# tuna2134/sbv2-api

Measured on NVIDIA B200. Metric: audio-sec/sec, higher is better.
Workload: dtype f16 operands / f32 accumulate on tcgen05 (decoder, flow; text encoder with two-term fp16 splits); f32 elsewhere

## Files before the change

### sbv2-api_b200/csrc/flow_attention_tc.cu

```cuda
#include <cuda_fp16.h>
#include <math_constants.h>

#include "kernels.h"

namespace sbv2 {
namespace {

constexpr int QT = 128, KT = 128, D = 96, DP = D / 8, RP = 16;
constexpr uint32_t TILE_BYTES = DP * KT * 16;
constexpr uint32_t P_BYTES = (KT / 8) * QT * 16;
constexpr uint32_t PREL_BYTES = (RP / 8) * QT * 16;
constexpr uint32_t REL_BYTES = DP * RP * 16;
constexpr int TM_O = 0, TM_SREL = 96, TM_S = 128 , TM_COLS = 512;
constexpr int NKV = 3;
constexpr int NSM_WARPS = 8;

__device__ __forceinline__ uint32_t smem_u32(const void* p) { return (uint32_t)__cvta_generic_to_shared(p); }
__device__ __forceinline__ void mbar_init(uint32_t bar, uint32_t count) {
  asm volatile("mbarrier.init.shared::cta.b64 [%0], %1;" ::"r"(bar), "r"(count));
}
__device__ __forceinline__ void mbar_expect_tx(uint32_t bar, uint32_t bytes) {
  asm volatile("mbarrier.arrive.expect_tx.shared::cta.b64 _, [%0], %1;" ::"r"(bar), "r"(bytes) : "memory");
}
__device__ __forceinline__ void mbar_arrive(uint32_t bar) {
  asm volatile("mbarrier.arrive.shared::cta.b64 _, [%0];" ::"r"(bar) : "memory");
}
__device__ __forceinline__ void mbar_wait(uint32_t bar, uint32_t parity) {
  asm volatile(
      "{\n"
      ".reg .pred P1;\n"
      "LAB_WAIT:\n"
      "mbarrier.try_wait.parity.shared::cta.b64 P1, [%0], %1, %2;\n"
      "@P1 bra DONE;\n"
      "bra LAB_WAIT;\n"
      "DONE:\n"
      "}\n" ::"r"(bar),
      "r"(parity), "r"(0x989680u)
      : "memory");
}
__device__ __forceinline__ void bulk_g2s(uint32_t dst, const void* src, uint32_t bytes, uint32_t bar) {
  asm volatile("cp.async.bulk.shared::cluster.global.mbarrier::complete_tx::bytes [%0], [%1], %2, [%3];" ::"r"(dst), "l"(src),
               "r"(bytes), "r"(bar)
               : "memory");
}
__device__ __forceinline__ void tc_fence_before() { asm volatile("tcgen05.fence::before_thread_sync;" ::: "memory"); }
__device__ __forceinline__ void tc_fence_after() { asm volatile("tcgen05.fence::after_thread_sync;" ::: "memory"); }
__device__ __forceinline__ void tc_commit(uint32_t bar) {
  asm volatile("tcgen05.commit.cta_group::1.mbarrier::arrive::one.shared::cluster.b64 [%0];" ::"r"(bar) : "memory");
}
__device__ __forceinline__ void tc_mma_f16(uint32_t tmem_d, uint64_t adesc, uint64_t bdesc, uint32_t idesc, uint32_t accumulate) {
  asm volatile(
      "{\n"
      ".reg .pred p;\n"
      "setp.ne.b32 p, %4, 0;\n"
      "tcgen05.mma.cta_group::1.kind::f16 [%0], %1, %2, %3, p;\n"
      "}\n" ::"r"(tmem_d),
      "l"(adesc), "l"(bdesc), "r"(idesc), "r"(accumulate)
      : "memory");
}
__device__ __forceinline__ void tc_ld32(uint32_t taddr, uint32_t* v) {
  asm volatile(
      "tcgen05.ld.sync.aligned.32x32b.x32.b32 "
      "{%0,%1,%2,%3,%4,%5,%6,%7,%8,%9,%10,%11,%12,%13,%14,%15,%16,%17,%18,%19,%20,%21,%22,%23,%24,%25,%26,%27,%28,%29,%30,%31}, [%32];"
      : "=r"(v[0]), "=r"(v[1]), "=r"(v[2]), "=r"(v[3]), "=r"(v[4]), "=r"(v[5]), "=r"(v[6]), "=r"(v[7]), "=r"(v[8]), "=r"(v[9]),
        "=r"(v[10]), "=r"(v[11]), "=r"(v[12]), "=r"(v[13]), "=r"(v[14]), "=r"(v[15]), "=r"(v[16]), "=r"(v[17]), "=r"(v[18]),
        "=r"(v[19]), "=r"(v[20]), "=r"(v[21]), "=r"(v[22]), "=r"(v[23]), "=r"(v[24]), "=r"(v[25]), "=r"(v[26]), "=r"(v[27]),
        "=r"(v[28]), "=r"(v[29]), "=r"(v[30]), "=r"(v[31])
      : "r"(taddr)
      : "memory");
}
__device__ __forceinline__ void tc_ld16(uint32_t taddr, uint32_t* v) {
  asm volatile(
      "tcgen05.ld.sync.aligned.32x32b.x16.b32 {%0,%1,%2,%3,%4,%5,%6,%7,%8,%9,%10,%11,%12,%13,%14,%15}, [%16];"
      : "=r"(v[0]), "=r"(v[1]), "=r"(v[2]), "=r"(v[3]), "=r"(v[4]), "=r"(v[5]), "=r"(v[6]), "=r"(v[7]), "=r"(v[8]), "=r"(v[9]),
        "=r"(v[10]), "=r"(v[11]), "=r"(v[12]), "=r"(v[13]), "=r"(v[14]), "=r"(v[15])
      : "r"(taddr)
      : "memory");
}
__device__ __forceinline__ void tc_wait_ld() { asm volatile("tcgen05.wait::ld.sync.aligned;" ::: "memory"); }
__device__ __forceinline__ uint32_t elect_one_sync() {
  uint32_t pred = 0;
  asm volatile(
      "{\n"
      ".reg .b32 %%rx;\n"
      ".reg .pred %%px;\n"
      "elect.sync %%rx|%%px, %1;\n"
      "@%%px mov.s32 %0, 1;\n"
      "}\n"
      : "+r"(pred)
      : "r"(0xffffffffu));
  return pred;
}
__device__ __forceinline__ float ex2_approx(float x) {
  float y;
  asm("ex2.approx.ftz.f32 %0, %1;" : "=f"(y) : "f"(x));
  return y;
}
__device__ __forceinline__ uint64_t make_desc(uint32_t saddr, uint32_t lbo_bytes, uint32_t sbo_bytes) {
  return (uint64_t)((saddr >> 4) & 0x3FFF) | ((uint64_t)((lbo_bytes >> 4) & 0x3FFF) << 16) | ((uint64_t)((sbo_bytes >> 4) & 0x3FFF) << 32) |
         ((uint64_t)1 << 46);
}
constexpr uint32_t idesc_f16(int n, int b_mn_major) {
  return (1u << 4) | ((uint32_t)b_mn_major << 16) | ((uint32_t)(n >> 3) << 17) | ((uint32_t)(128 >> 4) << 24);
}

#define ATRACE(ev, i)                                                                                   \
  do {                                                                                                   \
    if (trace != nullptr && blockIdx.x == 0 && blockIdx.y == 0 && blockIdx.z == 0 && (i) < 64) trace[(i) * 8 + (ev)] = clock64(); \
  } while (0)

__global__ void __launch_bounds__(288, 1) flow_attention_tc_kernel(__half* out, const __half* qkv, const __half* rel_k_p,
                                                                    const __half* rel_v_p, int heads, int window, PlanarSegs s,
                                                                    long long* trace) {
  extern __shared__ __align__(128) uint8_t smem[];
  const int warp = __shfl_sync(0xffffffffu, (int)(threadIdx.x >> 5), 0), lane = threadIdx.x & 31;
  const int b = s.order ? s.order[blockIdx.z] : (int)blockIdx.z, h = blockIdx.y;
  const int len = s.len[b];
  const int q0 = blockIdx.x * QT;
  if (q0 >= len) return;
  const long long pbase = s.pstart[b];
  const int n_kt = (len + KT - 1) / KT;

  const uint32_t sQ = smem_u32(smem);
  const uint32_t sK0 = sQ + TILE_BYTES;
  const uint32_t sV0 = sK0 + NKV * TILE_BYTES;
  const uint32_t sP = sV0 + NKV * TILE_BYTES;
  const uint32_t sPrel = sP + P_BYTES;
  const uint32_t sEk = sPrel + PREL_BYTES;
  const uint32_t sEv = sEk + REL_BYTES;
  const uint32_t sBar = sEv + REL_BYTES;
  const uint32_t bar_q = sBar, bar_kv = sBar + 8 , bar_kvfree = sBar + 40 , bar_s = sBar + 72 ,
                 bar_sfree = sBar + 88 , bar_p = sBar + 104, bar_pfree = sBar + 112, bar_done = sBar + 120;
  const uint32_t tmem_slot = sBar + 128;
  float* ml_x = reinterpret_cast<float*>(smem + (sBar - sQ) + 256);
  volatile uint32_t* tmem_slot_ptr = reinterpret_cast<volatile uint32_t*>(smem + (tmem_slot - sQ));

  if (threadIdx.x == 0) {
    mbar_init(bar_q, 1);
    for (int i = 0; i < NKV; ++i) {
      mbar_init(bar_kv + 8 * i, 1);
      mbar_init(bar_kvfree + 8 * i, 1);
    }
    mbar_init(bar_s, 1);
    mbar_init(bar_s + 8, 1);
    mbar_init(bar_sfree, 32 * NSM_WARPS);
    mbar_init(bar_sfree + 8, 32 * NSM_WARPS);
    mbar_init(bar_p, 32 * NSM_WARPS);
    mbar_init(bar_pfree, 1);
    mbar_init(bar_done, 1);
    asm volatile("fence.mbarrier_init.release.cluster;" ::: "memory");
  }
  if (warp == NSM_WARPS) {
    asm volatile("tcgen05.alloc.cta_group::1.sync.aligned.shared::cta.b32 [%0], %1;" ::"r"(tmem_slot), "r"((uint32_t)TM_COLS) : "memory");
    asm volatile("tcgen05.relinquish_alloc_permit.cta_group::1.sync.aligned;" ::: "memory");
  }
  if (threadIdx.x < 128) {
    const uint4 z = make_uint4(0, 0, 0, 0);
    *reinterpret_cast<uint4*>(smem + (sPrel - sQ) + threadIdx.x * 16) = z;
    *reinterpret_cast<uint4*>(smem + (sPrel - sQ) + QT * 16 + threadIdx.x * 16) = z;
  }
  asm volatile("fence.proxy.async.shared::cta;" ::: "memory");
  tc_fence_before();
  __syncthreads();
  tc_fence_after();
  const uint32_t tmem = *tmem_slot_ptr;
  pdl_launch_dependents();
  pdl_wait();

  const int q_plane0 = h * DP, k_plane0 = heads * DP + h * DP, v_plane0 = 2 * heads * DP + h * DP;
  const int n_tiles_total = 2 * n_kt;

  if (warp == NSM_WARPS) {
    auto load_tile = [&](int i) {
      const int buf = i % NKV;
      const uint32_t par = ((i / NKV) & 1) ^ 1;
      const int kt = i < n_kt ? i : i - n_kt;
      const bool with_v = i >= n_kt;
      const long long row0 = pbase + (long long)kt * KT;
      mbar_wait(bar_kvfree + 8 * buf, par);
      if (lane == 0) mbar_expect_tx(bar_kv + 8 * buf, with_v ? 2 * TILE_BYTES : TILE_BYTES);
      __syncwarp();
      if (lane < DP) {
        bulk_g2s(sK0 + buf * TILE_BYTES + lane * KT * 16, qkv + (size_t)(k_plane0 + lane) * s.plane_stride + row0 * 8, KT * 16,
                 bar_kv + 8 * buf);
      } else if (lane < 2 * DP && with_v) {
        const int pl = lane - DP;
        bulk_g2s(sV0 + buf * TILE_BYTES + pl * KT * 16, qkv + (size_t)(v_plane0 + pl) * s.plane_stride + row0 * 8, KT * 16,
                 bar_kv + 8 * buf);
      }
      __syncwarp();
    };
    if (elect_one_sync()) {
      mbar_expect_tx(bar_q, TILE_BYTES + 2 * REL_BYTES);
      for (int pl = 0; pl < DP; ++pl)
        bulk_g2s(sQ + pl * QT * 16, qkv + (size_t)(q_plane0 + pl) * s.plane_stride + (pbase + q0) * 8, QT * 16, bar_q);
      bulk_g2s(sEk, rel_k_p, REL_BYTES, bar_q);
      bulk_g2s(sEv, rel_v_p, REL_BYTES, bar_q);
    }
    __syncwarp();
    for (int i = 0; i < NKV && i < n_tiles_total; ++i) load_tile(i);
    mbar_wait(bar_q, 0);
    tc_fence_after();
    const uint64_t dq = make_desc(sQ, QT * 16, 128);
    const uint64_t dek = make_desc(sEk, RP * 16, 128);
    const uint64_t dp = make_desc(sP, QT * 16, 128);
    const uint64_t dprel = make_desc(sPrel, QT * 16, 128);
    const uint64_t dev = make_desc(sEv, 128, RP * 16);
    constexpr uint32_t ID_S = idesc_f16(KT, 0), ID_REL = idesc_f16(RP, 0), ID_O = idesc_f16(D, 1);
    if (elect_one_sync()) {
      for (int k = 0; k < D / 16; ++k)
        tc_mma_f16(tmem + TM_SREL, dq + (uint64_t)(k * 2 * QT), dek + (uint64_t)(k * 2 * RP), ID_REL, k > 0 ? 1u : 0u);
    }
    __syncwarp();
    auto issue_s = [&](int i) {
      const int sb = i & 1, kb = i % NKV;
      mbar_wait(bar_kv + 8 * kb, (i / NKV) & 1);
      if (lane == 0) ATRACE(0, i);
      mbar_wait(bar_sfree + 8 * sb, ((i >> 1) & 1) ^ 1);
      tc_fence_after();
      if (lane == 0) ATRACE(1, i);
      const uint64_t dk = make_desc(sK0 + kb * TILE_BYTES, KT * 16, 128);
      if (elect_one_sync()) {
        for (int k = 0; k < D / 16; ++k)
          tc_mma_f16(tmem + TM_S + sb * KT, dq + (uint64_t)(k * 2 * QT), dk + (uint64_t)(k * 2 * KT), ID_S, k > 0 ? 1u : 0u);
        tc_commit(bar_s + 8 * sb);
        if (i < n_kt) tc_commit(bar_kvfree + 8 * kb);
      }
      __syncwarp();
    };
    issue_s(0);
    for (int i = 0; i < n_tiles_total; ++i) {
      const int kb = i % NKV;
      if (i + 1 < n_tiles_total) issue_s(i + 1);
      if (i >= n_kt) {
        const int j = i - n_kt;
        mbar_wait(bar_p, j & 1);
        tc_fence_after();
        if (lane == 0) ATRACE(2, i);
        const uint64_t dv = make_desc(sV0 + kb * TILE_BYTES, 128, KT * 16);
        if (elect_one_sync()) {
          for (int k = 0; k < KT / 16; ++k)
            tc_mma_f16(tmem + TM_O, dp + (uint64_t)(k * 2 * QT), dv + (uint64_t)(k * 16), ID_O, (j > 0 || k > 0) ? 1u : 0u);
          tc_commit(bar_pfree);
          tc_commit(bar_kvfree + 8 * kb);
        }
        __syncwarp();
      }
      if (i + NKV < n_tiles_total) load_tile(i + NKV);
      if (lane == 0) ATRACE(3, i);
    }
    if (elect_one_sync()) {
      tc_mma_f16(tmem + TM_O, dprel, dev, ID_O, 1u);
      tc_commit(bar_done);
    }
    __syncwarp();
  } else {
    const int quarter = warp & 3, half = warp >> 2;
    const int row = quarter * 32 + lane;
    const int qi = q0 + row;
    const uint32_t lane_addr = tmem + ((uint32_t)(quarter * 32) << 16);
    const float c_scale = 1.4426950408889634f / sqrtf((float)D);
    float srel[9];
    {
      mbar_wait(bar_s, 0);
      tc_fence_after();
      uint32_t v[16];
      tc_ld16(lane_addr + TM_SREL, v);
      tc_wait_ld();
#pragma unroll
      for (int r = 0; r < 9; ++r) srel[r] = __uint_as_float(v[r]) * c_scale;
    }
    float m2 = -CUDART_INF_F, l = 0.f, mb = 0.f;
    uint8_t* prow = smem + (sP - sQ) + row * 16;
    uint8_t* prel_row = smem + (sPrel - sQ) + row * 16;
    auto pass_a = [&](const float* x, float c) {
      float mx = x[0];
#pragma unroll
      for (int e = 1; e < 32; ++e) mx = fmaxf(mx, x[e]);
      m2 = fmaxf(m2, mx * c);
    };
    auto pass_b_store = [&](const float* x, float c, int c32, float* pv) {
      float sum = 0.f;
#pragma unroll
      for (int e = 0; e < 32; ++e) {
        pv[e] = ex2_approx(fmaf(x[e], c, -mb));
        sum += pv[e];
      }
      l += sum;
#pragma unroll
      for (int q = 0; q < 4; ++q) {
        uint4 u;
        __half2* uh = reinterpret_cast<__half2*>(&u);
#pragma unroll
        for (int e = 0; e < 4; ++e) uh[e] = __floats2half2_rn(pv[q * 8 + 2 * e], pv[q * 8 + 2 * e + 1]);
        *reinterpret_cast<uint4*>(prow + (size_t)(c32 * 4 + q) * QT * 16) = u;
      }
    };
    for (int i = 0; i < n_tiles_total; ++i) {
      const bool pass_b = i >= n_kt;
      const int kt = pass_b ? i - n_kt : i;
      const int k0 = kt * KT;
      const int buf = i & 1;
      if (i > 0) {
        mbar_wait(bar_s + 8 * buf, (i >> 1) & 1);
        tc_fence_after();
      }
      if (threadIdx.x == 0) ATRACE(4, i);
      if (i == n_kt) {
        ml_x[(half * QT + row) * 2] = m2;
        asm volatile("bar.sync 1, %0;" ::"r"(32 * NSM_WARPS) : "memory");
        mb = fmaxf(m2, ml_x[((half ^ 1) * QT + row) * 2]);
      }
      if (pass_b && kt > 0) mbar_wait(bar_pfree, (kt - 1) & 1);
      if (threadIdx.x == 0) ATRACE(5, i);
#pragma unroll 1
      for (int cc = 0; cc < KT / 64; ++cc) {
        const int c = half * (KT / 64) + cc;
        const int kc0 = k0 + c * 32;
        if (kc0 >= len) {
          if (pass_b) {
            const uint4 z = make_uint4(0, 0, 0, 0);
#pragma unroll
            for (int q = 0; q < 4; ++q) *reinterpret_cast<uint4*>(prow + (size_t)(c * 4 + q) * QT * 16) = z;
          }
          continue;
        }
        uint32_t v[32];
        tc_ld32(lane_addr + TM_S + buf * KT + c * 32, v);
        tc_wait_ld();
        float* x = reinterpret_cast<float*>(v);
        const int j0 = kc0 - qi + 4;
        const bool band = j0 <= 8 && j0 + 31 >= 0;
        const bool tail = kc0 + 32 > len;
        if (!__any_sync(0xffffffffu, band) && !tail) {
          if (!pass_b) {
            pass_a(x, c_scale);
          } else {
            float pv[32];
            pass_b_store(x, c_scale, c, pv);
          }
          continue;
        }
#pragma unroll
        for (int e = 0; e < 32; ++e) {
          const int r = j0 + e;
          float add = 0.f;
#pragma unroll
          for (int rr = 0; rr < 9; ++rr) add = (r == rr) ? srel[rr] : add;
          x[e] = (kc0 + e < len) ? fmaf(x[e], c_scale, add) : -CUDART_INF_F;
        }
        if (!pass_b) {
          pass_a(x, 1.0f);
        } else {
          float pv[32];
          pass_b_store(x, 1.0f, c, pv);
#pragma unroll
          for (int rr = 0; rr < 9; ++rr) {
            const int e = rr - j0;
            float val = 0.f;
#pragma unroll
            for (int ee = 0; ee < 32; ++ee) val = (e == ee) ? pv[ee] : val;
            if (e >= 0 && e < 32) *reinterpret_cast<__half*>(prel_row + (size_t)(rr >> 3) * QT * 16 + (rr & 7) * 2) = __float2half_rn(val);
          }
        }
      }
      if (threadIdx.x == 0) ATRACE(6, i);
      tc_fence_before();
      mbar_arrive(bar_sfree + 8 * buf);
      if (pass_b) {
        asm volatile("fence.proxy.async.shared::cta;" ::: "memory");
        mbar_arrive(bar_p);
      }
    }
    ml_x[(half * QT + row) * 2 + 1] = l;
    asm volatile("bar.sync 1, %0;" ::"r"(32 * NSM_WARPS) : "memory");
    const float inv_l = 1.0f / (l + ml_x[((half ^ 1) * QT + row) * 2 + 1]);
    mbar_wait(bar_done, 0);
    tc_fence_after();
#pragma unroll 1
    for (int c = half * 2; c < (half == 0 ? 2 : D / 32); ++c) {
      uint32_t v[32];
      tc_ld32(lane_addr + TM_O + c * 32, v);
      tc_wait_ld();
      if (qi < len) {
#pragma unroll
        for (int q = 0; q < 4; ++q) {
          uint4 u;
          __half2* uh = reinterpret_cast<__half2*>(&u);
#pragma unroll
          for (int e = 0; e < 4; ++e)
            uh[e] = __floats2half2_rn(__uint_as_float(v[q * 8 + 2 * e]) * inv_l, __uint_as_float(v[q * 8 + 2 * e + 1]) * inv_l);
          *reinterpret_cast<uint4*>(out + (size_t)(h * DP + c * 4 + q) * s.plane_stride + (pbase + qi) * 8) = u;
        }
      }
    }
  }
  tc_fence_before();
  __syncthreads();
  if (warp == NSM_WARPS) {
    asm volatile("tcgen05.dealloc.cta_group::1.sync.aligned.b32 %0, %1;" ::"r"(tmem), "r"((uint32_t)TM_COLS) : "memory");
  }
}

}

std::vector<__half> pack_flow_rel_table(const float* table, int window, int head_dim) {
  const int R = 2 * window + 1;
  if (head_dim != D || R > RP) fail(SBV2_ERR_UNSUPPORTED, "tensor-core attention: head_dim must be 96 and window at most 7");
  std::vector<__half> pk(size_t(DP) * RP * 8, __float2half(0.f));
  for (int r = 0; r < R; ++r)
    for (int d = 0; d < D; ++d) pk[(size_t(d / 8) * RP + r) * 8 + d % 8] = __float2half_rn(table[size_t(r) * D + d]);
  return pk;
}

void launch_flow_attention_tc(const LaunchCtx& ctx, __half* ctx_out, const __half* qkv, const __half* rel_k_p, const __half* rel_v_p,
                              int heads, int head_dim, int window, const PlanarSegs& s, long long* trace) {
  if (s.n <= 0 || s.max_len <= 0) return;
  if (head_dim != D || window != 4) fail(SBV2_ERR_UNSUPPORTED, "tensor-core attention: head_dim must be 96 and window 4");
  const size_t smem = (1 + 2 * NKV) * TILE_BYTES + P_BYTES + PREL_BYTES + 2 * REL_BYTES + 256 + 2 * QT * 2 * 4;
  static PerDeviceOnce attr_once;
  attr_once.run([&] { CUDA_CHECK(cudaFuncSetAttribute(flow_attention_tc_kernel, cudaFuncAttributeMaxDynamicSharedMemorySize, (int)smem)); });
  dim3 grid((s.max_len + QT - 1) / QT, heads, s.n);
  launch_pdl(ctx.pdl, flow_attention_tc_kernel, grid, dim3(32 * (NSM_WARPS + 1)), smem, ctx.stream, ctx_out, qkv, rel_k_p, rel_v_p, heads, window, s,
             trace);
  ctx.count();
}

}

#ifdef SBV2_DEBUG_HOOKS
#include "model.h"
#include "umma_conv.h"
extern "C" int sbv2_debug_attn_trace(int T, int n_utt, int heads, long long* out_trace , float* out_ms) {
  using namespace sbv2;
  return guarded([&] {
    sbv2_model owner;
    owner.device = 0;
    CUDA_CHECK(cudaSetDevice(0));
    CUDA_CHECK(cudaStreamCreateWithFlags(&owner.stream, cudaStreamNonBlocking));
    LaunchCtx ctx = owner.ctx();
    DBuf meta, qkv, out, tr, rel;
    PinnedBuf pin;
    for (DBuf* b : {&meta, &qkv, &out, &tr, &rel}) b->stream = owner.stream;
    std::vector<int> ystart, ylen, muls{1};
    for (int i = 0; i < n_utt; ++i) {
      ystart.push_back(i * T);
      ylen.push_back(T);
    }
    BatchGeom bg = build_geoms(&owner, meta, pin, ystart, ylen, muls);
    const Geom& G = bg.g[0];
    const int C = heads * D;
    qkv.ensure(size_t(G.rows_tot) * 3 * C * 2);
    out.ensure(size_t(G.rows_tot) * C * 2);
    rel.ensure(2 * REL_BYTES);
    tr.ensure(64 * 8 * 8);
    CUDA_CHECK(cudaMemsetAsync(qkv.p, 0x11, size_t(G.rows_tot) * 3 * C * 2, owner.stream));
    CUDA_CHECK(cudaMemsetAsync(rel.p, 0, 2 * REL_BYTES, owner.stream));
    CUDA_CHECK(cudaMemsetAsync(tr.p, 0, 64 * 8 * 8, owner.stream));
    PlanarSegs ps;
    ps.start = bg.d_ystart;
    ps.pstart = G.d_pstart;
    ps.len = G.d_len;
    ps.n = n_utt;
    ps.max_len = T;
    ps.plane_stride = G.rows_tot * 8;
    const __half* rk = rel.as<__half>();
    const __half* rv = rk + REL_BYTES / 2;
    for (int i = 0; i < 2; ++i) launch_flow_attention_tc(ctx, out.as<__half>(), qkv.as<__half>(), rk, rv, heads, D, 4, ps, nullptr);
    cudaEvent_t e0, e1;
    CUDA_CHECK(cudaEventCreate(&e0));
    CUDA_CHECK(cudaEventCreate(&e1));
    CUDA_CHECK(cudaEventRecord(e0, owner.stream));
    for (int i = 0; i < 5; ++i) launch_flow_attention_tc(ctx, out.as<__half>(), qkv.as<__half>(), rk, rv, heads, D, 4, ps, nullptr);
    CUDA_CHECK(cudaEventRecord(e1, owner.stream));
    launch_flow_attention_tc(ctx, out.as<__half>(), qkv.as<__half>(), rk, rv, heads, D, 4, ps, tr.as<long long>());
    CUDA_CHECK(cudaStreamSynchronize(owner.stream));
    float ms = 0.f;
    CUDA_CHECK(cudaEventElapsedTime(&ms, e0, e1));
    if (out_ms) *out_ms = ms / 5.f;
    cudaEventDestroy(e0);
    cudaEventDestroy(e1);
    if (out_trace) CUDA_CHECK(cudaMemcpy(out_trace, tr.p, 64 * 8 * 8, cudaMemcpyDeviceToHost));
  });
}
#endif
```

Before: 9069.

## Rewrite flow attention as single-pass online softmax with two query tiles per CTA

Replaces the two-pass softmax, which computed S twice to find the max before forming P, with a single-pass online softmax. The O accumulator is rescaled in TMEM only when the running max grows by more than a threshold. Each CTA now processes two 128-row query tiles that share the K/V loads, and each warpgroup owns one tile instead of splitting columns across halves. The relative-position PV MMA moves into the per-step band tiles. This halves QK^T work and K reloads and removes cross-warp reductions, at the cost of TMEM load/store rescales, heavier register use (128-wide S per thread), and fewer CTAs in the grid.

```diff
diff --git a/sbv2-api_b200/csrc/flow_attention_tc.cu b/sbv2-api_b200/csrc/flow_attention_tc.cu
--- a/sbv2-api_b200/csrc/flow_attention_tc.cu
+++ b/sbv2-api_b200/csrc/flow_attention_tc.cu
@@ -11,9 +11,13 @@
 constexpr uint32_t P_BYTES = (KT / 8) * QT * 16;
 constexpr uint32_t PREL_BYTES = (RP / 8) * QT * 16;
 constexpr uint32_t REL_BYTES = DP * RP * 16;
-constexpr int TM_O = 0, TM_SREL = 96, TM_S = 128 , TM_COLS = 512;
-constexpr int NKV = 3;
+constexpr int TM_S = 0, TM_O = 256, TM_SREL = 448, TM_COLS = 512;
+constexpr uint32_t SM_Q = 0, SM_K = SM_Q + 2 * TILE_BYTES, SM_V = SM_K + 2 * TILE_BYTES, SM_P = SM_V + 2 * TILE_BYTES,
+                   SM_PREL = SM_P + 2 * P_BYTES, SM_EK = SM_PREL + 2 * PREL_BYTES, SM_EV = SM_EK + REL_BYTES, SM_BAR = SM_EV + REL_BYTES,
+                   SMEM_BYTES = SM_BAR + 256;
+static_assert(SMEM_BYTES <= 232448, "more than the 227 KB of shared memory a block may use");
 constexpr int NSM_WARPS = 8;
+constexpr float RESCALE_LOG2 = 8.f;
 
 __device__ __forceinline__ uint32_t smem_u32(const void* p) { return (uint32_t)__cvta_generic_to_shared(p); }
 __device__ __forceinline__ void mbar_init(uint32_t bar, uint32_t count) {
@@ -78,6 +82,16 @@
       : "memory");
 }
 __device__ __forceinline__ void tc_wait_ld() { asm volatile("tcgen05.wait::ld.sync.aligned;" ::: "memory"); }
+__device__ __forceinline__ void tc_st32(uint32_t taddr, const uint32_t* v) {
+  asm volatile(
+      "tcgen05.st.sync.aligned.32x32b.x32.b32 [%0], "
+      "{%1,%2,%3,%4,%5,%6,%7,%8,%9,%10,%11,%12,%13,%14,%15,%16,%17,%18,%19,%20,%21,%22,%23,%24,%25,%26,%27,%28,%29,%30,%31,%32};" ::"r"(taddr),
+      "r"(v[0]), "r"(v[1]), "r"(v[2]), "r"(v[3]), "r"(v[4]), "r"(v[5]), "r"(v[6]), "r"(v[7]), "r"(v[8]), "r"(v[9]), "r"(v[10]), "r"(v[11]),
+      "r"(v[12]), "r"(v[13]), "r"(v[14]), "r"(v[15]), "r"(v[16]), "r"(v[17]), "r"(v[18]), "r"(v[19]), "r"(v[20]), "r"(v[21]), "r"(v[22]),
+      "r"(v[23]), "r"(v[24]), "r"(v[25]), "r"(v[26]), "r"(v[27]), "r"(v[28]), "r"(v[29]), "r"(v[30]), "r"(v[31])
+      : "memory");
+}
+__device__ __forceinline__ void tc_wait_st() { asm volatile("tcgen05.wait::st.sync.aligned;" ::: "memory"); }
 __device__ __forceinline__ uint32_t elect_one_sync() {
   uint32_t pred = 0;
   asm volatile(
@@ -109,55 +123,50 @@
     if (trace != nullptr && blockIdx.x == 0 && blockIdx.y == 0 && blockIdx.z == 0 && (i) < 64) trace[(i) * 8 + (ev)] = clock64(); \
   } while (0)
 
-__global__ void __launch_bounds__(288, 1) flow_attention_tc_kernel(__half* out, const __half* qkv, const __half* rel_k_p,
-                                                                    const __half* rel_v_p, int heads, int window, PlanarSegs s,
-                                                                    long long* trace) {
+__global__ void __launch_bounds__(32 * (NSM_WARPS + 1), 1) flow_attention_tc_kernel(__half* out, const __half* qkv, const __half* rel_k_p,
+                                                                                    const __half* rel_v_p, int heads, int window, PlanarSegs s,
+                                                                                    long long* trace) {
   extern __shared__ __align__(128) uint8_t smem[];
   const int warp = __shfl_sync(0xffffffffu, (int)(threadIdx.x >> 5), 0), lane = threadIdx.x & 31;
   const int b = s.order ? s.order[blockIdx.z] : (int)blockIdx.z, h = blockIdx.y;
   const int len = s.len[b];
-  const int q0 = blockIdx.x * QT;
-  if (q0 >= len) return;
+  const int tA = 2 * blockIdx.x;
+  if (tA * QT >= len) return;
+  const bool has_b = (tA + 1) * QT < len;
+  const int n_qt = has_b ? 2 : 1;
   const long long pbase = s.pstart[b];
   const int n_kt = (len + KT - 1) / KT;
 
-  const uint32_t sQ = smem_u32(smem);
-  const uint32_t sK0 = sQ + TILE_BYTES;
-  const uint32_t sV0 = sK0 + NKV * TILE_BYTES;
-  const uint32_t sP = sV0 + NKV * TILE_BYTES;
-  const uint32_t sPrel = sP + P_BYTES;
-  const uint32_t sEk = sPrel + PREL_BYTES;
-  const uint32_t sEv = sEk + REL_BYTES;
-  const uint32_t sBar = sEv + REL_BYTES;
-  const uint32_t bar_q = sBar, bar_kv = sBar + 8 , bar_kvfree = sBar + 40 , bar_s = sBar + 72 ,
-                 bar_sfree = sBar + 88 , bar_p = sBar + 104, bar_pfree = sBar + 112, bar_done = sBar + 120;
-  const uint32_t tmem_slot = sBar + 128;
-  float* ml_x = reinterpret_cast<float*>(smem + (sBar - sQ) + 256);
-  volatile uint32_t* tmem_slot_ptr = reinterpret_cast<volatile uint32_t*>(smem + (tmem_slot - sQ));
+  const uint32_t s0 = smem_u32(smem);
+  const uint32_t bar = s0 + SM_BAR;
+  const uint32_t bar_q = bar, bar_kfull = bar + 8, bar_kfree = bar + 24, bar_vfull = bar + 40, bar_vfree = bar + 56, bar_s = bar + 72,
+                 bar_sfree = bar + 88, bar_p = bar + 104, bar_pfree = bar + 120;
+  const uint32_t tmem_slot = bar + 136;
+  volatile uint32_t* tmem_slot_ptr = reinterpret_cast<volatile uint32_t*>(smem + SM_BAR + 136);
 
   if (threadIdx.x == 0) {
     mbar_init(bar_q, 1);
-    for (int i = 0; i < NKV; ++i) {
-      mbar_init(bar_kv + 8 * i, 1);
-      mbar_init(bar_kvfree + 8 * i, 1);
-    }
-    mbar_init(bar_s, 1);
-    mbar_init(bar_s + 8, 1);
-    mbar_init(bar_sfree, 32 * NSM_WARPS);
-    mbar_init(bar_sfree + 8, 32 * NSM_WARPS);
-    mbar_init(bar_p, 32 * NSM_WARPS);
-    mbar_init(bar_pfree, 1);
-    mbar_init(bar_done, 1);
+    for (int i = 0; i < 2; ++i) {
+      mbar_init(bar_kfull + 8 * i, 1);
+      mbar_init(bar_kfree + 8 * i, 1);
+      mbar_init(bar_vfull + 8 * i, 1);
+      mbar_init(bar_vfree + 8 * i, 1);
+      mbar_init(bar_s + 8 * i, 1);
+      mbar_init(bar_sfree + 8 * i, QT);
+      mbar_init(bar_p + 8 * i, QT);
+      mbar_init(bar_pfree + 8 * i, 1);
+    }
     asm volatile("fence.mbarrier_init.release.cluster;" ::: "memory");
   }
   if (warp == NSM_WARPS) {
     asm volatile("tcgen05.alloc.cta_group::1.sync.aligned.shared::cta.b32 [%0], %1;" ::"r"(tmem_slot), "r"((uint32_t)TM_COLS) : "memory");
     asm volatile("tcgen05.relinquish_alloc_permit.cta_group::1.sync.aligned;" ::: "memory");
   }
-  if (threadIdx.x < 128) {
+  if (threadIdx.x < 2 * QT) {
     const uint4 z = make_uint4(0, 0, 0, 0);
-    *reinterpret_cast<uint4*>(smem + (sPrel - sQ) + threadIdx.x * 16) = z;
-    *reinterpret_cast<uint4*>(smem + (sPrel - sQ) + QT * 16 + threadIdx.x * 16) = z;
+    uint8_t* p = smem + SM_PREL + (threadIdx.x / QT) * PREL_BYTES + (threadIdx.x % QT) * 16;
+    *reinterpret_cast<uint4*>(p) = z;
+    *reinterpret_cast<uint4*>(p + QT * 16) = z;
   }
   asm volatile("fence.proxy.async.shared::cta;" ::: "memory");
   tc_fence_before();
@@ -168,219 +177,225 @@
   pdl_wait();
 
   const int q_plane0 = h * DP, k_plane0 = heads * DP + h * DP, v_plane0 = 2 * heads * DP + h * DP;
-  const int n_tiles_total = 2 * n_kt;
 
   if (warp == NSM_WARPS) {
-    auto load_tile = [&](int i) {
-      const int buf = i % NKV;
-      const uint32_t par = ((i / NKV) & 1) ^ 1;
-      const int kt = i < n_kt ? i : i - n_kt;
-      const bool with_v = i >= n_kt;
-      const long long row0 = pbase + (long long)kt * KT;
-      mbar_wait(bar_kvfree + 8 * buf, par);
-      if (lane == 0) mbar_expect_tx(bar_kv + 8 * buf, with_v ? 2 * TILE_BYTES : TILE_BYTES);
+    auto load_tile = [&](int j, uint32_t full, uint32_t free_, uint32_t dst, int plane0) {
+      const int slot = j & 1;
+      if (j >= 2) mbar_wait(free_ + 8 * slot, ((j >> 1) & 1) ^ 1);
+      if (lane == 0) mbar_expect_tx(full + 8 * slot, TILE_BYTES);
       __syncwarp();
-      if (lane < DP) {
-        bulk_g2s(sK0 + buf * TILE_BYTES + lane * KT * 16, qkv + (size_t)(k_plane0 + lane) * s.plane_stride + row0 * 8, KT * 16,
-                 bar_kv + 8 * buf);
-      } else if (lane < 2 * DP && with_v) {
-        const int pl = lane - DP;
-        bulk_g2s(sV0 + buf * TILE_BYTES + pl * KT * 16, qkv + (size_t)(v_plane0 + pl) * s.plane_stride + row0 * 8, KT * 16,
-                 bar_kv + 8 * buf);
-      }
+      if (lane < DP)
+        bulk_g2s(dst + slot * TILE_BYTES + lane * KT * 16, qkv + (size_t)(plane0 + lane) * s.plane_stride + (pbase + (long long)j * KT) * 8,
+                 KT * 16, full + 8 * slot);
       __syncwarp();
     };
     if (elect_one_sync()) {
-      mbar_expect_tx(bar_q, TILE_BYTES + 2 * REL_BYTES);
-      for (int pl = 0; pl < DP; ++pl)
-        bulk_g2s(sQ + pl * QT * 16, qkv + (size_t)(q_plane0 + pl) * s.plane_stride + (pbase + q0) * 8, QT * 16, bar_q);
-      bulk_g2s(sEk, rel_k_p, REL_BYTES, bar_q);
-      bulk_g2s(sEv, rel_v_p, REL_BYTES, bar_q);
+      mbar_expect_tx(bar_q, n_qt * TILE_BYTES + 2 * REL_BYTES);
+      for (int t = 0; t < n_qt; ++t)
+        for (int pl = 0; pl < DP; ++pl)
+          bulk_g2s(s0 + SM_Q + t * TILE_BYTES + pl * QT * 16,
+                   qkv + (size_t)(q_plane0 + pl) * s.plane_stride + (pbase + (long long)(tA + t) * QT) * 8, QT * 16, bar_q);
+      bulk_g2s(s0 + SM_EK, rel_k_p, REL_BYTES, bar_q);
+      bulk_g2s(s0 + SM_EV, rel_v_p, REL_BYTES, bar_q);
     }
     __syncwarp();
-    for (int i = 0; i < NKV && i < n_tiles_total; ++i) load_tile(i);
+    for (int j = 0; j < 2 && j < n_kt; ++j) {
+      load_tile(j, bar_kfull, bar_kfree, s0 + SM_K, k_plane0);
+      load_tile(j, bar_vfull, bar_vfree, s0 + SM_V, v_plane0);
+    }
     mbar_wait(bar_q, 0);
     tc_fence_after();
-    const uint64_t dq = make_desc(sQ, QT * 16, 128);
-    const uint64_t dek = make_desc(sEk, RP * 16, 128);
-    const uint64_t dp = make_desc(sP, QT * 16, 128);
-    const uint64_t dprel = make_desc(sPrel, QT * 16, 128);
-    const uint64_t dev = make_desc(sEv, 128, RP * 16);
+    const uint64_t dek = make_desc(s0 + SM_EK, RP * 16, 128);
+    const uint64_t dev = make_desc(s0 + SM_EV, 128, RP * 16);
     constexpr uint32_t ID_S = idesc_f16(KT, 0), ID_REL = idesc_f16(RP, 0), ID_O = idesc_f16(D, 1);
     if (elect_one_sync()) {
-      for (int k = 0; k < D / 16; ++k)
-        tc_mma_f16(tmem + TM_SREL, dq + (uint64_t)(k * 2 * QT), dek + (uint64_t)(k * 2 * RP), ID_REL, k > 0 ? 1u : 0u);
+      for (int t = 0; t < n_qt; ++t) {
+        const uint64_t dq = make_desc(s0 + SM_Q + t * TILE_BYTES, QT * 16, 128);
+        for (int k = 0; k < D / 16; ++k)
+          tc_mma_f16(tmem + TM_SREL + t * RP, dq + (uint64_t)(k * 2 * QT), dek + (uint64_t)(k * 2 * RP), ID_REL, k > 0 ? 1u : 0u);
+      }
     }
     __syncwarp();
-    auto issue_s = [&](int i) {
-      const int sb = i & 1, kb = i % NKV;
-      mbar_wait(bar_kv + 8 * kb, (i / NKV) & 1);
-      if (lane == 0) ATRACE(0, i);
-      mbar_wait(bar_sfree + 8 * sb, ((i >> 1) & 1) ^ 1);
-      tc_fence_after();
-      if (lane == 0) ATRACE(1, i);
-      const uint64_t dk = make_desc(sK0 + kb * TILE_BYTES, KT * 16, 128);
-      if (elect_one_sync()) {
-        for (int k = 0; k < D / 16; ++k)
-          tc_mma_f16(tmem + TM_S + sb * KT, dq + (uint64_t)(k * 2 * QT), dk + (uint64_t)(k * 2 * KT), ID_S, k > 0 ? 1u : 0u);
-        tc_commit(bar_s + 8 * sb);
-        if (i < n_kt) tc_commit(bar_kvfree + 8 * kb);
-      }
-      __syncwarp();
+    auto issue_s = [&](int j) {
+      const int slot = j & 1;
+      mbar_wait(bar_kfull + 8 * slot, (j >> 1) & 1);
+      const uint64_t dk = make_desc(s0 + SM_K + slot * TILE_BYTES, KT * 16, 128);
+      for (int t = 0; t < n_qt; ++t) {
+        if (j > 0) mbar_wait(bar_sfree + 8 * t, (j - 1) & 1);
+        tc_fence_after();
+        if (lane == 0) ATRACE(t, j);
+        const uint64_t dq = make_desc(s0 + SM_Q + t * TILE_BYTES, QT * 16, 128);
+        if (elect_one_sync()) {
+          for (int k = 0; k < D / 16; ++k)
+            tc_mma_f16(tmem + TM_S + t * KT, dq + (uint64_t)(k * 2 * QT), dk + (uint64_t)(k * 2 * KT), ID_S, k > 0 ? 1u : 0u);
+          tc_commit(bar_s + 8 * t);
+          if (t == n_qt - 1) tc_commit(bar_kfree + 8 * slot);
+        }
+        __syncwarp();
+      }
+    };
+    auto issue_pv = [&](int j) {
+      const int slot = j & 1;
+      mbar_wait(bar_vfull + 8 * slot, (j >> 1) & 1);
+      const uint64_t dv = make_desc(s0 + SM_V + slot * TILE_BYTES, 128, KT * 16);
+      for (int t = 0; t < n_qt; ++t) {
+        mbar_wait(bar_p + 8 * t, j & 1);
+        tc_fence_after();
+        if (lane == 0) ATRACE(2 + t, j);
+        const int dt = j - (tA + t);
+        const uint64_t dp = make_desc(s0 + SM_P + t * P_BYTES, QT * 16, 128);
+        if (elect_one_sync()) {
+          for (int k = 0; k < KT / 16; ++k)
+            tc_mma_f16(tmem + TM_O + t * D, dp + (uint64_t)(k * 2 * QT), dv + (uint64_t)(k * 16), ID_O, (j > 0 || k > 0) ? 1u : 0u);
+          if (dt >= -1 && dt <= 1) tc_mma_f16(tmem + TM_O + t * D, make_desc(s0 + SM_PREL + t * PREL_BYTES, QT * 16, 128), dev, ID_O, 1u);
+          tc_commit(bar_pfree + 8 * t);
+          if (t == n_qt - 1) tc_commit(bar_vfree + 8 * slot);
+        }
+        __syncwarp();
+      }
     };
     issue_s(0);
-    for (int i = 0; i < n_tiles_total; ++i) {
-      const int kb = i % NKV;
-      if (i + 1 < n_tiles_total) issue_s(i + 1);
-      if (i >= n_kt) {
-        const int j = i - n_kt;
-        mbar_wait(bar_p, j & 1);
-        tc_fence_after();
-        if (lane == 0) ATRACE(2, i);
-        const uint64_t dv = make_desc(sV0 + kb * TILE_BYTES, 128, KT * 16);
-        if (elect_one_sync()) {
-          for (int k = 0; k < KT / 16; ++k)
-            tc_mma_f16(tmem + TM_O, dp + (uint64_t)(k * 2 * QT), dv + (uint64_t)(k * 16), ID_O, (j > 0 || k > 0) ? 1u : 0u);
-          tc_commit(bar_pfree);
-          tc_commit(bar_kvfree + 8 * kb);
-        }
-        __syncwarp();
-      }
-      if (i + NKV < n_tiles_total) load_tile(i + NKV);
-      if (lane == 0) ATRACE(3, i);
-    }
-    if (elect_one_sync()) {
-      tc_mma_f16(tmem + TM_O, dprel, dev, ID_O, 1u);
-      tc_commit(bar_done);
-    }
-    __syncwarp();
-  } else {
-    const int quarter = warp & 3, half = warp >> 2;
+    for (int j = 0; j < n_kt; ++j) {
+      if (j + 1 < n_kt) issue_s(j + 1);
+      if (j + 2 < n_kt) load_tile(j + 2, bar_kfull, bar_kfree, s0 + SM_K, k_plane0);
+      if (j >= 1 && j + 1 < n_kt) load_tile(j + 1, bar_vfull, bar_vfree, s0 + SM_V, v_plane0);
+      issue_pv(j);
+    }
+  } else if (warp < 4 || has_b) {
+    const int t = warp >> 2, quarter = warp & 3;
     const int row = quarter * 32 + lane;
-    const int qi = q0 + row;
+    const int qi = (tA + t) * QT + row;
     const uint32_t lane_addr = tmem + ((uint32_t)(quarter * 32) << 16);
+    const uint32_t tm_s = lane_addr + TM_S + t * KT, tm_o = lane_addr + TM_O + t * D;
+    const uint32_t bs = bar_s + 8 * t, bsfree = bar_sfree + 8 * t, bp = bar_p + 8 * t, bpfree = bar_pfree + 8 * t;
     const float c_scale = 1.4426950408889634f / sqrtf((float)D);
     float srel[9];
     {
-      mbar_wait(bar_s, 0);
+      mbar_wait(bs, 0);
       tc_fence_after();
       uint32_t v[16];
-      tc_ld16(lane_addr + TM_SREL, v);
+      tc_ld16(lane_addr + TM_SREL + t * RP, v);
       tc_wait_ld();
 #pragma unroll
       for (int r = 0; r < 9; ++r) srel[r] = __uint_as_float(v[r]) * c_scale;
     }
-    float m2 = -CUDART_INF_F, l = 0.f, mb = 0.f;
-    uint8_t* prow = smem + (sP - sQ) + row * 16;
-    uint8_t* prel_row = smem + (sPrel - sQ) + row * 16;
-    auto pass_a = [&](const float* x, float c) {
-      float mx = x[0];
-#pragma unroll
-      for (int e = 1; e < 32; ++e) mx = fmaxf(mx, x[e]);
-      m2 = fmaxf(m2, mx * c);
-    };
-    auto pass_b_store = [&](const float* x, float c, int c32, float* pv) {
-      float sum = 0.f;
-#pragma unroll
-      for (int e = 0; e < 32; ++e) {
-        pv[e] = ex2_approx(fmaf(x[e], c, -mb));
-        sum += pv[e];
-      }
-      l += sum;
-#pragma unroll
-      for (int q = 0; q < 4; ++q) {
-        uint4 u;
-        __half2* uh = reinterpret_cast<__half2*>(&u);
-#pragma unroll
-        for (int e = 0; e < 4; ++e) uh[e] = __floats2half2_rn(pv[q * 8 + 2 * e], pv[q * 8 + 2 * e + 1]);
-        *reinterpret_cast<uint4*>(prow + (size_t)(c32 * 4 + q) * QT * 16) = u;
-      }
-    };
-    for (int i = 0; i < n_tiles_total; ++i) {
-      const bool pass_b = i >= n_kt;
-      const int kt = pass_b ? i - n_kt : i;
-      const int k0 = kt * KT;
-      const int buf = i & 1;
-      if (i > 0) {
-        mbar_wait(bar_s + 8 * buf, (i >> 1) & 1);
+    float m = -CUDART_INF_F, l = 0.f;
+    uint8_t* prow = smem + SM_P + t * P_BYTES + row * 16;
+    uint8_t* prel_row = smem + SM_PREL + t * PREL_BYTES + row * 16;
+#pragma unroll 1
+    for (int j = 0; j < n_kt; ++j) {
+      const int k0 = j * KT;
+      if (j > 0) {
+        mbar_wait(bs, j & 1);
         tc_fence_after();
       }
-      if (threadIdx.x == 0) ATRACE(4, i);
-      if (i == n_kt) {
-        ml_x[(half * QT + row) * 2] = m2;
-        asm volatile("bar.sync 1, %0;" ::"r"(32 * NSM_WARPS) : "memory");
-        mb = fmaxf(m2, ml_x[((half ^ 1) * QT + row) * 2]);
-      }
-      if (pass_b && kt > 0) mbar_wait(bar_pfree, (kt - 1) & 1);
-      if (threadIdx.x == 0) ATRACE(5, i);
-#pragma unroll 1
-      for (int cc = 0; cc < KT / 64; ++cc) {
-        const int c = half * (KT / 64) + cc;
+      if (row == 0) ATRACE(4 + 2 * t, j);
+      uint32_t v[KT];
+#pragma unroll
+      for (int c = 0; c < KT / 32; ++c) tc_ld32(tm_s + c * 32, v + c * 32);
+      tc_wait_ld();
+      tc_fence_before();
+      mbar_arrive(bsfree);
+      float* x = reinterpret_cast<float*>(v);
+      float cs[KT / 32], mt = -CUDART_INF_F;
+      bool bandc[KT / 32];
+#pragma unroll
+      for (int c = 0; c < KT / 32; ++c) {
         const int kc0 = k0 + c * 32;
-        if (kc0 >= len) {
-          if (pass_b) {
-            const uint4 z = make_uint4(0, 0, 0, 0);
-#pragma unroll
-            for (int q = 0; q < 4; ++q) *reinterpret_cast<uint4*>(prow + (size_t)(c * 4 + q) * QT * 16) = z;
+        const int j0 = kc0 - qi + 4;
+        bandc[c] = __any_sync(0xffffffffu, j0 <= 8 && j0 + 31 >= 0);
+        cs[c] = c_scale;
+        if (bandc[c] || kc0 + 32 > len) {
+#pragma unroll
+          for (int e = 0; e < 32; ++e) {
+            const int r = j0 + e;
+            float add = 0.f;
+#pragma unroll
+            for (int rr = 0; rr < 9; ++rr) add = (r == rr) ? srel[rr] : add;
+            x[c * 32 + e] = (kc0 + e < len) ? fmaf(x[c * 32 + e], c_scale, add) : -CUDART_INF_F;
           }
-          continue;
-        }
-        uint32_t v[32];
-        tc_ld32(lane_addr + TM_S + buf * KT + c * 32, v);
-        tc_wait_ld();
-        float* x = reinterpret_cast<float*>(v);
-        const int j0 = kc0 - qi + 4;
-        const bool band = j0 <= 8 && j0 + 31 >= 0;
-        const bool tail = kc0 + 32 > len;
-        if (!__any_sync(0xffffffffu, band) && !tail) {
-          if (!pass_b) {
-            pass_a(x, c_scale);
-          } else {
-            float pv[32];
-            pass_b_store(x, c_scale, c, pv);
-          }
-          continue;
-        }
-#pragma unroll
-        for (int e = 0; e < 32; ++e) {
-          const int r = j0 + e;
-          float add = 0.f;
-#pragma unroll
-          for (int rr = 0; rr < 9; ++rr) add = (r == rr) ? srel[rr] : add;
-          x[e] = (kc0 + e < len) ? fmaf(x[e], c_scale, add) : -CUDART_INF_F;
-        }
-        if (!pass_b) {
-          pass_a(x, 1.0f);
-        } else {
-          float pv[32];
-          pass_b_store(x, 1.0f, c, pv);
+          cs[c] = 1.f;
+        }
+        float mx = x[c * 32];
+#pragma unroll
+        for (int e = 1; e < 32; ++e) mx = fmaxf(mx, x[c * 32 + e]);
+        mt = fmaxf(mt, mx * cs[c]);
+      }
+      const bool grow = mt > m + RESCALE_LOG2;
+      float scale = 1.f;
+      if (grow) {
+        scale = ex2_approx(m - mt);
+        m = mt;
+      }
+      uint32_t ph[KT / 2];
+      float sum[KT / 32];
+#pragma unroll
+      for (int c = 0; c < KT / 32; ++c) {
+        sum[c] = 0.f;
+#pragma unroll
+        for (int e = 0; e < 16; ++e) {
+          const float p0 = ex2_approx(fmaf(x[c * 32 + 2 * e], cs[c], -m)), p1 = ex2_approx(fmaf(x[c * 32 + 2 * e + 1], cs[c], -m));
+          sum[c] += p0;
+          sum[c] += p1;
+          const __half2 hp = __floats2half2_rn(p0, p1);
+          ph[c * 16 + e] = *reinterpret_cast<const uint32_t*>(&hp);
+        }
+      }
+      l = l * scale + ((sum[0] + sum[1]) + (sum[2] + sum[3]));
+      const int dt = j - (tA + t);
+      const bool band_step = dt >= -1 && dt <= 1;
+      uint32_t prel[9];
+#pragma unroll
+      for (int rr = 0; rr < 9; ++rr) prel[rr] = 0u;
+      if (band_step) {
+#pragma unroll
+        for (int c = 0; c < KT / 32; ++c) {
+          if (!bandc[c]) continue;
+          const int j0 = k0 + c * 32 - qi + 4;
 #pragma unroll
           for (int rr = 0; rr < 9; ++rr) {
             const int e = rr - j0;
-            float val = 0.f;
-#pragma unroll
-            for (int ee = 0; ee < 32; ++ee) val = (e == ee) ? pv[ee] : val;
-            if (e >= 0 && e < 32) *reinterpret_cast<__half*>(prel_row + (size_t)(rr >> 3) * QT * 16 + (rr & 7) * 2) = __float2half_rn(val);
+#pragma unroll
+            for (int ee = 0; ee < 32; ++ee) prel[rr] = (e == ee) ? (ph[c * 16 + ee / 2] >> (16 * (ee & 1))) & 0xFFFFu : prel[rr];
           }
         }
       }
-      if (threadIdx.x == 0) ATRACE(6, i);
+      if (j > 0) {
+        mbar_wait(bpfree, (j - 1) & 1);
+        tc_fence_after();
+      }
+#pragma unroll
+      for (int q = 0; q < KT / 8; ++q)
+        *reinterpret_cast<uint4*>(prow + (size_t)q * QT * 16) = make_uint4(ph[4 * q], ph[4 * q + 1], ph[4 * q + 2], ph[4 * q + 3]);
+      if (band_step) {
+        *reinterpret_cast<uint4*>(prel_row) =
+            make_uint4(prel[0] | prel[1] << 16, prel[2] | prel[3] << 16, prel[4] | prel[5] << 16, prel[6] | prel[7] << 16);
+        *reinterpret_cast<uint16_t*>(prel_row + QT * 16) = (uint16_t)prel[8];
+      }
+      if (j > 0 && __any_sync(0xffffffffu, grow)) {
+#pragma unroll 1
+        for (int c = 0; c < D / 32; ++c) {
+          uint32_t o[32];
+          tc_ld32(tm_o + c * 32, o);
+          tc_wait_ld();
+#pragma unroll
+          for (int e = 0; e < 32; ++e) o[e] = __float_as_uint(__uint_as_float(o[e]) * scale);
+          tc_st32(tm_o + c * 32, o);
+        }
+        tc_wait_st();
+      }
+      asm volatile("fence.proxy.async.shared::cta;" ::: "memory");
       tc_fence_before();
-      mbar_arrive(bar_sfree + 8 * buf);
-      if (pass_b) {
-        asm volatile("fence.proxy.async.shared::cta;" ::: "memory");
-        mbar_arrive(bar_p);
-      }
-    }
-    ml_x[(half * QT + row) * 2 + 1] = l;
-    asm volatile("bar.sync 1, %0;" ::"r"(32 * NSM_WARPS) : "memory");
-    const float inv_l = 1.0f / (l + ml_x[((half ^ 1) * QT + row) * 2 + 1]);
-    mbar_wait(bar_done, 0);
+      mbar_arrive(bp);
+      if (row == 0) ATRACE(5 + 2 * t, j);
+    }
+    const float inv_l = 1.0f / l;
+    mbar_wait(bpfree, (n_kt - 1) & 1);
     tc_fence_after();
 #pragma unroll 1
-    for (int c = half * 2; c < (half == 0 ? 2 : D / 32); ++c) {
+    for (int c = 0; c < D / 32; ++c) {
       uint32_t v[32];
-      tc_ld32(lane_addr + TM_O + c * 32, v);
+      tc_ld32(tm_o + c * 32, v);
       tc_wait_ld();
       if (qi < len) {
 #pragma unroll
@@ -417,10 +432,10 @@
                               int heads, int head_dim, int window, const PlanarSegs& s, long long* trace) {
   if (s.n <= 0 || s.max_len <= 0) return;
   if (head_dim != D || window != 4) fail(SBV2_ERR_UNSUPPORTED, "tensor-core attention: head_dim must be 96 and window 4");
-  const size_t smem = (1 + 2 * NKV) * TILE_BYTES + P_BYTES + PREL_BYTES + 2 * REL_BYTES + 256 + 2 * QT * 2 * 4;
+  const size_t smem = SMEM_BYTES;
   static PerDeviceOnce attr_once;
   attr_once.run([&] { CUDA_CHECK(cudaFuncSetAttribute(flow_attention_tc_kernel, cudaFuncAttributeMaxDynamicSharedMemorySize, (int)smem)); });
-  dim3 grid((s.max_len + QT - 1) / QT, heads, s.n);
+  dim3 grid((s.max_len + 2 * QT - 1) / (2 * QT), heads, s.n);
   launch_pdl(ctx.pdl, flow_attention_tc_kernel, grid, dim3(32 * (NSM_WARPS + 1)), smem, ctx.stream, ctx_out, qkv, rel_k_p, rel_v_p, heads, window, s,
              trace);
   ctx.count();
```

Result: slower. 8866, median of 6 (-2.2%).
